# KoslickiLab/YACHT

Measured on AMD Instinct MI355X. Metric: ref-sketch containment queries/sec (yacht run), higher is better.
Workload: dtype u64

## Files before the change

yacht_amd/csrc/yh_api.hip:

```cpp
#include "yh_common.h"
#include "yh_abund.h"
#include "yh_explain.h"
#include "yh_sort.h"
#include "yh_pack.h"

#include <mutex>
#include <unordered_map>

#include <stdarg.h>
#include <string.h>
#include <time.h>

#include <algorithm>
#include <utility>
#include <vector>

static thread_local char g_err[1024] = "";

void yh_set_error(const char* fmt, ...) {
    va_list ap;
    va_start(ap, fmt);
    vsnprintf(g_err, sizeof(g_err), fmt, ap);
    va_end(ap);
}
// ... 546 lines not shown
        return db_create_common(nullptr, v.offsets, false, v.n_refs, device_id, flags, out, &v);
    } catch (const std::bad_alloc&) {
        yh_set_error("yh_db_create_packed: out of host memory");
        return YH_ERR_OOM;
    } catch (const std::exception& ex) {
        yh_set_error("yh_db_create_packed: %s", ex.what());
        return YH_ERR_INVALID_ARG;
    }
}

int yh_db_destroy(yh_db* db) {
    if (!db) return YH_OK;
    if (db->device >= 0) (void)hipSetDevice(db->device);
    if (db->fin_stream) (void)hipStreamSynchronize(db->fin_stream);
    if (db->stream) (void)hipStreamSynchronize(db->stream);
    if (db->ev_fin) (void)hipEventDestroy(db->ev_fin);
    for (yh_db::BatchSlot& bs : db->batch) if (bs.ev_first) (void)hipEventDestroy(bs.ev_first);
    if (db->tmp_psort) { yh_psort_destroy(db, db->tmp_psort); db->tmp_psort = nullptr; }
    if (db->ctx_bits[0]) {
        db->d_maskbits = db->ctx_bits[0];
        db->d_work = db->ctx_work[0];
        db->d_work_count = db->ctx_count[0];
        for (int c = 1; c < YH_RUN_CONTEXTS; ++c) {
            yh_dfree(db, db->ctx_bits[c]);
            yh_dfree(db, db->ctx_work[c]);
            yh_dfree(db, db->ctx_count[c]);
        }
    }
    void* ptrs[] = {db->d_values, db->d_offsets, db->d_sizes, db->d_g, db->d_po, db->d_pr, db->d_pg, db->d_nshared,
                    db->d_dh, db->d_dref, db->d_dir, db->d_bkt, db->d_cbkt, db->d_ovf_keys, db->d_ovf_vals,
                    db->d_rpo, db->d_rg, db->d_rrec, db->d_rrecx, db->d_filter, db->d_hrec, db->d_hrecx, db->d_hmult, db->d_hpo,
                    db->d_work, db->d_work_count, db->d_mask, db->d_maskbits, db->d_hit, db->d_excl_e, db->d_overlap_tmp,
                    db->d_sample_tmp, db->d_out_tmp, db->d_flag, db->d_reps, db->batch[0].d_scratch, db->batch[1].d_scratch, db->batch[2].d_scratch, db->d_sdelta, db->d_shdr, db->d_srec,
                    db->d_wg_key, db->d_ghost_src, db->d_bad_word, db->d_prank, db->d_fz_rec, db->d_fz_list, db->d_fz_list2, db->d_fz_off, db->d_fz_tab};
    for (void* p : ptrs)
        if (p) yh_dfree(db, p);
    for (auto& pair : db->ev_xfer)
        for (hipEvent_t e : pair) if (e) (void)hipEventDestroy(e);
    ring_destroy(db->ev_overlap);
    ring_destroy(db->ev_excl);
    ring_destroy(db->ev_pair);
    for (hipStream_t q : db->st_in) if (q) (void)hipStreamSynchronize(q);
    for (RunSlot& s : db->slots) {
        yh_dfree(db, s.d_sample);
        yh_dfree(db, s.d_packed);
        yh_dfree(db, s.d_rows);
        yh_dfree(db, s.d_out);
        yh_dfree(db, s.d_bad);
        if (s.h_bad) (void)hipHostFree(s.h_bad);
        if (s.ev_up) (void)hipEventDestroy(s.ev_up);
        if (s.ev_out) (void)hipEventDestroy(s.ev_out);
    }
    for (hipStream_t q : db->st_in) if (q) (void)hipStreamDestroy(q);
    if (db->stream) { (void)hipStreamSynchronize(db->stream); yh_pool_trim(db); }
    if (db->own_stream) (void)hipStreamDestroy(db->own_stream);
    free(db->h_pw_i);
    free(db->h_pw_j);
    free(db->h_pw_c);
    delete db;
    return YH_OK;
}

int yh_db_get_info(yh_db* db, yh_db_info* info) {
    if (!db_ok(db)) return YH_ERR_INVALID_ARG;
    if (!info) { yh_set_error("info is null"); return YH_ERR_INVALID_ARG; }
    memset(info, 0, sizeof(*info));
    info->n_refs = db->n_refs;
// ... 1010 lines not shown
```

yacht_amd/csrc/yh_batch.hip:

```cpp
#include "yh_common.h"

#include <stdlib.h>
#include <string.h>

#include <algorithm>
#include <vector>

namespace {

constexpr u32 BATCH_MAX = 256;
constexpr u32 BATCH_MAX_PLANES = BATCH_MAX / 64;
inline u32 planes_of(u32 n_samples) { return (n_samples + 63u) / 64u; }

constexpr int EXCL_BLOCK = 256;
inline u32 grid_for(u64 work_items, u32 block, u32 max_blocks = 16384) {
    u64 g = (work_items + block - 1) / block;
    if (g < 1) g = 1;
    if (g > max_blocks) g = max_blocks;
    return (u32)g;
}

#ifndef YH_BATCH_TILE
#define YH_BATCH_TILE 2048
#endif
constexpr u32 BATCH_TILE = YH_BATCH_TILE;
#ifndef YH_BATCH_U
#define YH_BATCH_U 1
#endif
constexpr int BATCH_U = YH_BATCH_U;

constexpr u32 BATCH_TBITS = 10;
__global__ void __launch_bounds__(256) k_batch_lookup(const u64* __restrict__ samples, const u64* __restrict__ soff,
                                                      u32 n_samples, const YhDirView dv, const u64* __restrict__ po,
                                                      const u32* __restrict__ pr, u64 n_refs,
                                                      u32* __restrict__ overlap , u32* __restrict__ ovsh ,
                                                      const u32* __restrict__ filter, u64 filter_mul) {
    constexpr u32 TSLOTS = 1u << BATCH_TBITS;
    __shared__ u64 off[BATCH_MAX + 1];
    __shared__ u64 s_max_nt;
    __shared__ u32 tkey[TSLOTS], tcnt[TSLOTS], tcnt2[TSLOTS];
    for (u32 q = threadIdx.x; q <= n_samples; q += 256) off[q] = soff[q];
    if (threadIdx.x == 0) s_max_nt = 0;
    __syncthreads();
    {
        u64 m = 0;
        if (threadIdx.x < 64)
            for (u32 q = threadIdx.x; q < n_samples; q += 64) m = max(m, (off[q + 1] - off[q] + BATCH_TILE - 1) / BATCH_TILE);
        if (threadIdx.x < 64 && m) atomicMax((unsigned long long*)&s_max_nt, (unsigned long long)m);
    }
    __syncthreads();
    const u64 max_nt = s_max_nt;
    const u64 n_slots = max_nt * n_samples;
    const u64 group = 8ull * n_samples;
    for (u64 c = blockIdx.x; c < (n_slots + group - 1) / group * group; c += gridDim.x) {
        const u64 l = c % group;
        const u64 v = (c / group) * 8 + (l & 7u);
        const u32 s = (u32)(l >> 3);
        if (v >= max_nt) continue;
        const u64 n_s = off[s + 1] - off[s], nt_s = (n_s + BATCH_TILE - 1) / BATCH_TILE;
        if (nt_s == 0) continue;
        const u64 i = v * nt_s / max_nt;
        if (v > 0 && (v - 1) * nt_s / max_nt == i) continue;
        for (u32 k = threadIdx.x; k < TSLOTS; k += 256) { tkey[k] = 0; tcnt[k] = 0; tcnt2[k] = 0; }
        __syncthreads();
        u32* row = overlap + (u64)s * n_refs;
        u32* row2 = ovsh + (u64)s * n_refs;
        auto add = [&](u32 ref, bool shared) {
#if defined(YH_ABLATE_BATCH) && YH_ABLATE_BATCH
            if (ref == 0x7ffffff1u) row[0] = 1;
            return;
#endif
            u32 slot = (ref * 2654435761u) >> (32 - BATCH_TBITS);
#if defined(YH_BATCH_DIRECT_ATOMICS) && YH_BATCH_DIRECT_ATOMICS
            atomicAdd(&row[ref], 1u);
            if (shared) atomicAdd(&row2[ref], 1u);
            return;
#endif
#pragma unroll 1
            for (int probe = 0; probe < 2; ++probe, slot = (slot + 1) & (TSLOTS - 1)) {
                const u32 old = atomicCAS(&tkey[slot], 0u, ref + 1);
                if (old == 0 || old == ref + 1) {
                    atomicAdd(&tcnt[slot], 1u);
                    if (shared) atomicAdd(&tcnt2[slot], 1u);
                    return;
                }
            }
            atomicAdd(&row[ref], 1u);
            if (shared) atomicAdd(&row2[ref], 1u);
        };
        const u64 k_end = min(n_s, (i + 1) * BATCH_TILE);
        auto hits_of = [&](u32 r) {
            if (r == YH_DIR_NONE) return;
            if (!(r & 0x80000000u)) {
                add(r, false);
            } else {
                const u32 gi = r & 0x7fffffffu;
                for (u64 q = po[gi], qe = po[gi + 1]; q < qe; ++q) add(pr[q], true);
            }
        };
        for (u64 k0 = i * BATCH_TILE; k0 < k_end; k0 += 256u * BATCH_U) {
            u64 h[BATCH_U];
            bool ok[BATCH_U];
            u32 w[BATCH_U];
            u64 bit[BATCH_U];
            YhDirView::v4u a[BATCH_U], b[BATCH_U], c[BATCH_U], d[BATCH_U];
#pragma unroll
            for (int u = 0; u < BATCH_U; ++u) {
                const u64 k = k0 + (u64)u * 256u + threadIdx.x;
#if defined(YH_BATCH_NT) && (YH_BATCH_NT & 2)
                h[u] = __builtin_nontemporal_load(&samples[off[s] + min(k, k_end - 1)]);
#else
                h[u] = samples[off[s] + min(k, k_end - 1)];
#endif
                ok[u] = k < k_end && h[u] <= dv.max_hash;
                if (!ok[u]) h[u] = 0;
            }
#if defined(YH_ABLATE_BATCH_READS) && (YH_ABLATE_BATCH_READS & 2)
            if (false) {
#else
            if (filter) {
#endif
#pragma unroll
                for (int u = 0; u < BATCH_U; ++u) {
                    bit[u] = yh_bucket_of(h[u], dv.bkt_lsh, filter_mul);
                    w[u] = filter[bit[u] >> 5];
                }
#pragma unroll
                for (int u = 0; u < BATCH_U; ++u) {
                    const u32 m = yh_filter_mask(h[u], bit[u]);
                    ok[u] = ok[u] && (w[u] & m) == m;
// ... 408 lines not shown
                   u32* d_overlap, u32* d_excl, u32* d_match, int phases, u64* d_maskword_out, const u64* d_gathered,
                   u32 n_ranks, int slot) {
    if (!db->has_dir || !db->has_index) {
        yh_set_error("yh_run_batch needs the directory of the distinct hashes (handle created with YH_DB_NO_DIRECTORY?)");
        return YH_ERR_UNSUPPORTED;
    }
    if (n_samples < 1 || n_samples > BATCH_MAX) { yh_set_error("1..%u samples per batch", BATCH_MAX); return YH_ERR_INVALID_ARG; }
    const u32 npl = planes_of(n_samples);
    const bool split_streams = db->fin_stream && phases != 3;
    hipStream_t st = (split_streams && phases == 2) ? db->fin_stream : db->stream;
    const u64 N = db->n_refs;
    if (N == 0) return YH_OK;
    const u64 BN = (u64)n_samples * N;
    const u64 G = db->n_shared;
    if (G && db->n_postings && !db->d_hrec) { yh_set_error("yh_run_batch needs the holder sets of the handle"); return YH_ERR_UNSUPPORTED; }
    yh_db::BatchSlot& bs = db->batch[slot];
    u64* d_maskword = nullptr;
    u32* d_ovsh = nullptr;
    u64 need = 0;
    YH_TRY(batch_slot_scratch(db, slot, (phases & 1) ? n_samples : std::max(n_samples, bs.n_samples), &d_maskword, &d_ovsh, &need));
    if (phases & 1) { bs.n_samples = n_samples; bs.words_valid = false; }
    if (phases & 1) {
    YH_HIP(hipMemsetAsync(d_overlap, 0, BN * sizeof(u32), st));
    if (!bs.ovsh_clean) YH_HIP(hipMemsetAsync(bs.d_scratch, 0, bs.cap, st));
    bs.ovsh_clean = false;
    yh_ring_record_begin(db, db->ev_overlap, st);
    if (total_hashes && db->n_distinct) {
        const u64 n_tiles = (total_hashes + BATCH_TILE - 1) / BATCH_TILE + n_samples;
        if (n_tiles >> 31) { yh_set_error("batch too large"); return YH_ERR_INVALID_ARG; }
        static const long grid_env = [] { const char* e = yh_tune_env("YH_BATCH_GRID"); return e ? atol(e) : -1L; }();
        const u64 grid_cap = grid_env < 0 ? 32768ull : grid_env == 0 ? (u64)0x7fffff00 : (u64)grid_env;
        k_batch_lookup<<<(u32)std::min<u64>((n_tiles + 7) / 8 * 8, grid_cap), 256, 0, st>>>(d_samples, d_soff, n_samples, yh_dir_view(db),
                                                                                       db->d_po, db->d_pr, N, d_overlap, d_ovsh,
                                                                                       yh_filter_of(db), db->filter_mul);
    }
    yh_ring_record_end(db, db->ev_overlap, st);
    hipStream_t sw = st;
    if (split_streams) {
        YH_HIP(hipEventRecord(bs.ev_first, st));
        sw = db->fin_stream;
        YH_HIP(hipStreamWaitEvent(sw, bs.ev_first, 0));
    }
    k_batch_maskwords<<<(u32)((N + 255) / 256), 256, 0, sw>>>(d_overlap, n_samples, N, d_maskword, split_streams ? nullptr : db->d_maskbits);
    if (d_maskword_out) YH_HIP(hipMemcpyAsync(d_maskword_out, d_maskword, (u64)npl * N * sizeof(u64), hipMemcpyDeviceToDevice, sw));
    if (split_streams) { YH_HIP(hipEventRecord(db->ev_fin, sw)); db->fin_pending = true; }
    }
    if (!(phases & 2)) { YH_HIP(hipGetLastError()); return YH_OK; }
    YH_HIP(hipMemsetAsync(d_excl, 0, BN * sizeof(u32), st));
    yh_ring_record_begin(db, db->ev_excl, st);
    if (d_gathered)
        k_batch_or_maskwords<<<(u32)((N + 255) / 256), 256, 0, st>>>(d_gathered, n_ranks, N, d_maskword, db->d_maskbits, npl);
    if (G && db->n_postings) {
        YH_HIP(hipMemsetAsync(db->d_work_count, 0, sizeof(u32), st));
        k_batch_worklist<<<(u32)((N + 255) / 256), 256, 0, st>>>(N, db->d_maskbits, db->d_hpo, db->d_work, db->d_work_count);
        const u32 sets_blocks = (u32)std::min<u64>(4096, ((u64)db->n_chunks + 3) / 4 + 1);
        k_batch_sets<<<sets_blocks, 256, 0, st>>>(db->d_work, db->d_work_count, db->d_hrec, db->d_hrecx, db->d_hmult, db->d_pr,
                                                   d_maskword, N, d_excl, npl);
    }
    static const bool dense_final = [] { const char* e = yh_tune_env("YH_BATCH_DENSE_FINAL"); return e && e[0] == '1'; }();
    if (dense_final) {
        k_batch_final<<<grid_for(BN, 256, 8192), 256, 0, st>>>(n_samples, N, db->d_sizes, db->d_nshared, d_overlap, d_ovsh,
                                                               d_excl, d_match, d_gathered ? d_maskword : nullptr);
    } else {
        YH_HIP(hipMemsetAsync(d_match, 0, BN * sizeof(u32), st));
        k_batch_final_sparse<<<(u32)((N + 255) / 256), 256, 0, st>>>(n_samples, N, npl, db->d_sizes, db->d_nshared, d_overlap, d_ovsh,
                                                                   d_excl, d_match, d_maskword);
    }
// ... 27 lines not shown
```

yacht_amd/csrc/yh_build.hip:

```cpp
#include "yh_common.h"
#include "yh_sort.h"
#include "yh_pack.h"

#include <rocprim/device/device_merge.hpp>
#include <rocprim/device/device_radix_sort.hpp>
#include <rocprim/device/device_scan.hpp>
#include <rocprim/iterator/counting_iterator.hpp>
#include <rocprim/iterator/transform_iterator.hpp>

#include <stdio.h>
#include <time.h>

#include <algorithm>
#include <atomic>
#include <thread>
#include <mutex>
#include <vector>

namespace {

constexpr int WAVE = 64;

__global__ void k_scan_refs(const u64* __restrict__ values, const u64* __restrict__ offsets, u64 n_refs,
                            u32* __restrict__ sizes, u32* __restrict__ flag, u64* __restrict__ maxv) {
// ... 324 lines not shown
            atomicAdd(&hcnt[pref[p]], 1u);
        }
    }
}

__global__ void k_chunk_counts(const u32* __restrict__ nshared, u64 n, u32* __restrict__ cc) {
    const u64 r = blockIdx.x * (u64)blockDim.x + threadIdx.x;
    if (r < n) cc[r] = (nshared[r] + (u32)(YH_EXCL_PIECE - 1)) / (u32)YH_EXCL_PIECE;
}
__global__ void k_fill_rg(u64 n_post, const u32* __restrict__ pr, const u32* __restrict__ pg, const u64* __restrict__ po,
                          const u32* __restrict__ rpo, u32* __restrict__ cursor, u32* __restrict__ rg,
                          uint4* __restrict__ rrec, uint4* __restrict__ rrecx, u32* __restrict__ pref) {
    for (u64 k = blockIdx.x * (u64)blockDim.x + threadIdx.x; k < n_post; k += (u64)gridDim.x * blockDim.x) {
        const u32 r = pr[k], g = pg[k];
        const u32 dst = rpo[r] + atomicAdd(&cursor[r], 1u);
        rg[dst] = g;
        if (pref) pref[dst] = r;
        if (rrec) {
            const u64 q0 = po[g], q1 = po[g + 1];
            uint4 rec, recx = make_uint4(0u, 0u, 0u, 0u);
            if (q1 - q0 <= 8) {
                u32 o[7] = {0u, 0u, 0u, 0u, 0u, 0u, 0u};
                u32 n = 0;
                for (u64 q = q0; q < q1; ++q)
                    if (q != k) o[n++] = pr[q];
                rec = make_uint4(o[0], o[1], o[2], n);
                recx = make_uint4(o[3], o[4], o[5], o[6]);
            } else {
                rec = make_uint4((u32)q0, (u32)(q1 - q0), 0u, 0xffffffffu);
            }
            rrec[dst] = rec;
            rrecx[dst] = recx;
        }
    }
}
__global__ void k_filter_build(const u64* __restrict__ dh, u64 n, u32 lsh, u64 fmul, u32* __restrict__ filter) {
    for (u64 i = blockIdx.x * (u64)blockDim.x + threadIdx.x; i < n; i += (u64)gridDim.x * blockDim.x) {
        const u64 bit = __umul64hi(dh[i] << lsh, fmul);
        atomicOr(&filter[bit >> 5], yh_filter_mask(dh[i], bit));
    }
}

inline u32 grid_for(u64 work_items, u32 block, u32 max_blocks = 16384) {
    u64 g = (work_items + block - 1) / block;
    if (g < 1) g = 1;
    if (g > max_blocks) g = max_blocks;
    return (u32)g;
}

}

static int validate_begin(yh_db* db) {
    const u64 N = db->n_refs;
    YH_TRY(yh_dmalloc(db, (void**)&db->d_sizes, std::max<u64>(N, 1) * sizeof(u32)));
    YH_TRY(yh_dmalloc(db, (void**)&db->d_flag, 32));
    YH_HIP(hipMemsetAsync(db->d_flag, 0, 32, db->stream));
    YH_HIP(hipMemsetAsync(db->d_sizes, 0, std::max<u64>(N, 1) * sizeof(u32), db->stream));
    return YH_OK;
}
static int validate_refs(yh_db* db, const u64* d_values, const u64* d_offsets, u64 r0, u64 r1) {
    if (r1 > r0) {
        u64* d_maxv = (u64*)(db->d_flag + 2);
        k_scan_refs<<<grid_for((r1 - r0) * WAVE, 256), 256, 0, db->stream>>>(d_values, d_offsets + r0, r1 - r0, db->d_sizes + r0,
                                                                            db->d_flag, d_maxv);
        YH_HIP(hipGetLastError());
    }
// ... 727 lines not shown
            IDX_HIP(hipMemsetAsync(db->d_ovf_keys, 0, cap * sizeof(u64), st));
            IDX_HIP(hipMemsetAsync(db->d_ovf_vals, 0xff, cap * sizeof(u32), st));
            if (rc == YH_OK)
                k_cbkt_build<<<grid_for(db->n_distinct, 256), 256, 0, st>>>(d_dh_tmp, d_dref_tmp, db->n_distinct, db->bkt_lsh, mul_c,
                                                                            reinterpret_cast<u32*>(db->d_cbkt), db->d_ovf_keys,
                                                                            db->d_ovf_vals, db->ovf_mask);
            IDX_HIP(hipGetLastError());
            static const u32 fbph = [] { const char* e = yh_tune_env("YH_FILTER_BPH"); return e ? (u32)atoi(e) : 4u; }();
            static const u64 fmin = [] { const char* e = yh_tune_env("YH_FILTER_MIN"); return e ? (u64)atoll(e) : (u64)(1u << 20); }();
            if (rc == YH_OK && fbph && db->n_distinct >= fmin) {
                const u64 fbits = ((db->n_distinct * fbph + 511) / 512) * 512;
                db->filter_mul = mul_for(fbits);
                db->filter_bits = fbits;
                rc = yh_dmalloc(db, (void**)&db->d_filter, fbits / 8 + 64);
                IDX_HIP(hipMemsetAsync(db->d_filter, 0, fbits / 8 + 64, st));
                if (rc == YH_OK && db->filter_mul)
                    k_filter_build<<<grid_for(db->n_distinct, 256), 256, 0, st>>>(d_dh_tmp, db->n_distinct, db->bkt_lsh, db->filter_mul,
                                                                                  db->d_filter);
                IDX_HIP(hipGetLastError());
            }
            IDX_HIP(hipStreamSynchronize(st));
        }
        IDX_HIP(hipStreamSynchronize(st));
        TRACE("index: emit + table + filter");
        yh_tfree(db, d_dh_tmp);
        yh_tfree(db, d_dref_tmp);
        if (rc == YH_OK && full) db->has_dir = true;
        if (rc == YH_OK && want_stream) rc = build_stream(db, d_sk, d_sv, d_elem_g, H);
        TRACE("index: delta stream");
        yh_tfree(db, d_elem_g);
        d_elem_g = nullptr;
        IDX_HIP(hipGetLastError());
        IDX_HIP(hipMemcpyAsync(db->d_po + db->n_shared, &db->n_postings, sizeof(u64), hipMemcpyHostToDevice, st));
        if (rc == YH_OK && db->n_postings && N && !(db->flags & YH_DB_PAIRWISE_ONLY)) {
            u32 *d_cc = nullptr, *d_cpo = nullptr, *d_cur = nullptr;
            void* d_st = nullptr;
            size_t st_bytes = 0;
            rc = yh_dmalloc(db, (void**)&db->d_rpo, (N + 1) * sizeof(u32));
            if (rc == YH_OK) rc = yh_dmalloc(db, (void**)&db->d_rg, db->n_postings * sizeof(u32));
            if (rc == YH_OK && want_stream) rc = yh_dmalloc(db, (void**)&db->d_rrec, (db->n_postings + 1) * sizeof(uint4));
            if (rc == YH_OK && want_stream) rc = yh_dmalloc(db, (void**)&db->d_rrecx, (db->n_postings + 1) * sizeof(uint4));
            IDX_HIP(yh_tmalloc(db, (void**)&d_cc, N * sizeof(u32)));
            IDX_HIP(yh_tmalloc(db, (void**)&d_cpo, (N + 1) * sizeof(u32)));
            IDX_HIP(yh_tmalloc(db, (void**)&d_cur, N * sizeof(u32)));
            IDX_HIP(rocprim::inclusive_scan(nullptr, st_bytes, db->d_nshared, db->d_rpo + 1, N, rocprim::plus<u32>(), st));
            IDX_HIP(yh_tmalloc(db, &d_st, st_bytes + 256));
            IDX_HIP(hipMemsetAsync(db->d_rpo, 0, sizeof(u32), st));
            IDX_HIP(hipMemsetAsync(d_cpo, 0, sizeof(u32), st));
            IDX_HIP(hipMemsetAsync(d_cur, 0, N * sizeof(u32), st));
            IDX_HIP(rocprim::inclusive_scan(d_st, st_bytes, db->d_nshared, db->d_rpo + 1, N, rocprim::plus<u32>(), st));
            if (rc == YH_OK) k_chunk_counts<<<(u32)((N + 255) / 256), 256, 0, st>>>(db->d_nshared, N, d_cc);
            IDX_HIP(rocprim::inclusive_scan(d_st, st_bytes, d_cc, d_cpo + 1, N, rocprim::plus<u32>(), st));
            u32 n_chunks = 0;
            IDX_HIP(hipMemcpyAsync(&n_chunks, d_cpo + N, sizeof(u32), hipMemcpyDeviceToHost, st));
            IDX_HIP(hipStreamSynchronize(st));
            db->n_chunks = n_chunks;
            if (rc == YH_OK) rc = yh_dmalloc(db, (void**)&db->d_work, ((u64)n_chunks + 64) * sizeof(uint4));
            if (rc == YH_OK) rc = yh_dmalloc(db, (void**)&db->d_work_count, 16);
            IDX_HIP(hipMemsetAsync(db->d_work_count, 0, 16, st));
            u32* d_pref = nullptr;
            if (want_stream) IDX_HIP(yh_tmalloc(db, (void**)&d_pref, db->n_postings * sizeof(u32)));
            if (rc == YH_OK)
                k_fill_rg<<<grid_for(db->n_postings, 256), 256, 0, st>>>(db->n_postings, db->d_pr, db->d_pg, db->d_po, db->d_rpo,
                                                                         d_cur, db->d_rg, db->d_rrec, db->d_rrecx, d_pref);
            IDX_HIP(hipGetLastError());
            if (trace_on()) { IDX_HIP(hipStreamSynchronize(st)); TRACE("index: reference-major view"); }
// ... 70 lines not shown
```

yacht_amd/csrc/yh_common.h:

```cpp
#pragma once

#include <hip/hip_runtime.h>
#include <stdint.h>
#include <stdio.h>
#include <string>
#include <vector>

#include "../../include/yacht_hip.h"

typedef unsigned long long u64;
typedef uint32_t u32;
typedef uint16_t u16;
typedef uint8_t u8;

static_assert(sizeof(u64) == sizeof(uint64_t), "u64 must be 64 bits");

void yh_set_error(const char* fmt, ...);

#define YH_HIP(call)                                                                        \
    do {                                                                                    \
        hipError_t e__ = (call);                                                            \
        if (e__ != hipSuccess) {                                                            \
            yh_set_error("%s failed: %s (%s:%d)", #call, hipGetErrorString(e__), __FILE__,  \
                         __LINE__);                                                         \
// ... 41 lines not shown
    u64 rows_cap = 0;
    bool rows_mode = false;
    u32* d_out = nullptr;
    u32* d_bad = nullptr;
    u32* h_bad = nullptr;
    u32* h_bad_dev = nullptr;
    hipEvent_t ev_up = nullptr, ev_out = nullptr;
    bool busy = false;
};

struct yh_db {
    int device = -1;
    uint32_t flags = 0;
    hipStream_t own_stream = nullptr;
    hipStream_t stream = nullptr;

    u64 n_refs = 0;
    u64 n_hashes = 0;
    u64 max_hash = 0;
    u64 device_bytes = 0;

    u64* d_values = nullptr;
    u64* d_offsets = nullptr;

    u32* d_sizes = nullptr;

    bool has_index = false;
    u64 n_distinct = 0;
    u64 n_shared = 0;
    u64 n_postings = 0;
    u64* d_g = nullptr;
    u64* d_po = nullptr;
    u32* d_pr = nullptr;
    u32* d_pg = nullptr;
    u32* d_prank = nullptr;
    u32* d_nshared = nullptr;
    bool fz = false;
    u64* d_fz_rec = nullptr;
    u32* d_fz_list = nullptr;
    u32* d_fz_list2 = nullptr;
    u64 fz_list_split = 0;
    u64 n_spilled_pairs = 0, n_spilled_buckets = 0;
    u32 sort_path = 0;
    u64* d_fz_off = nullptr;
    u32* d_fz_tab = nullptr;
    bool fz_nshared = false;

    u64* d_dh = nullptr;
    u32* d_dref = nullptr;
    u32* d_dir = nullptr;
    u32 dir_shift = 0, dir_nb = 0;
    u32* d_rpo = nullptr;
    u32* d_rg = nullptr;
    uint4* d_work = nullptr;
    u32* d_work_count = nullptr;
    uint4* d_rrec = nullptr;
    uint4* d_rrecx = nullptr;
    u32* d_filter = nullptr;
    u64 filter_mul = 0, filter_bits = 0;
    uint4* d_hrec = nullptr;
    uint4* d_hrecx = nullptr;
    u32* d_hmult = nullptr;
    u32* d_hpo = nullptr;
    u32 n_sets = 0;
    u32 n_chunks = 0;
    u8* d_sdelta = nullptr;
// ... 262 lines not shown
```

yacht_amd/csrc/yh_query.hip:

```cpp
#include "yh_common.h"

#include <stdlib.h>
#include <string.h>

#include <algorithm>
#include <vector>

namespace {

constexpr int WAVE = 64;
constexpr int EXCL_PIECE_C = YH_EXCL_PIECE;

typedef u64 u64x2 __attribute__((ext_vector_type(2)));

__device__ __forceinline__ u32 xcd_remap(u32 bid, u32 nwg) {
    const u32 q = nwg >> 3, r = nwg & 7u;
    const u32 xcd = bid & 7u;
    const u32 base = (xcd < r) ? xcd * (q + 1) : r * (q + 1) + (xcd - r) * q;
    return base + (bid >> 3);
}

#ifndef YH_XCD_ATOMICS
#define YH_XCD_ATOMICS 0
#endif
// ... 671 lines not shown
    for (u64 q = q0; q < qe; q += 4) {
        u32 h[4];
#pragma unroll
        for (int i = 0; i < 4; ++i) h[i] = pr[min(q + (u64)i, qe - 1)];
#pragma unroll
        for (int i = 0; i < 4; ++i)
            if (q + (u64)i < qe) add(h[i]);
    }
}

#ifndef YH_IDX_THREADS
#define YH_IDX_THREADS 1024
#endif
#ifndef YH_IDX_TBITS
#define YH_IDX_TBITS 10
#endif
constexpr int IDX_THREADS = YH_IDX_THREADS;
struct TileLookup {
    const u64* sample;
    u64 n;
    YhDirView dv;
    const u32* filter;
    u64 filter_mul;
    const u64* po;
    const u32* pr;
    u32* reps;
    u32 rep_mask;
    u64 n_refs;
    u8* hit;
    u32* reps2;
    u32* work_count;
    const u32* bad;
    u32 bad_gen;
};
template <int U, int THREADS, int TBITS>
__device__ __forceinline__ void lookup_tile_body(u32 wg, u32* tkey, u32* tcnt, u32* tcnt2, const TileLookup& q) {
    constexpr u32 TSLOTS = 1u << TBITS;
    const u64* __restrict__ sample = q.sample;
    const u64 n = q.n;
    const YhDirView& dv = q.dv;
    const u32* __restrict__ filter = q.filter;
    if (q.work_count && wg == 0 && threadIdx.x == 0) *q.work_count = 0;
    u32* my = q.reps + (u64)replica_of(wg, q.rep_mask) * q.n_refs;
    u32* my2 = q.reps2 ? q.reps2 + (u64)replica_of(wg, q.rep_mask) * q.n_refs : nullptr;
    const u64 base = wg * (u64)(THREADS * U);
    u64 h[U];
    bool ok[U];
#pragma unroll
    for (int u = 0; u < U; ++u) {
        const u64 t = base + (u64)u * THREADS + threadIdx.x;
        h[u] = sample[min(t, n - 1)];
        ok[u] = t < n && h[u] <= dv.max_hash;
        if (!ok[u]) h[u] = 0;
    }
#if !(defined(YH_ABLATE_LOOKUP) && (YH_ABLATE_LOOKUP & 32))
    if (q.bad && *q.bad == q.bad_gen) return;
#endif
    for (u32 k = threadIdx.x; k < TSLOTS; k += THREADS) { tkey[k] = 0; tcnt[k] = 0; tcnt2[k] = 0; }
    YhDirView::v4u a[U], b[U], c[U], d[U];
    u32 r[U];
#if defined(YH_ABLATE_LOOKUP) && (YH_ABLATE_LOOKUP & 16)
    if (false) {
#else
    if (filter) {
#endif
        u64 bit[U];
// ... 14 lines not shown
        for (int u = 0; u < U; ++u) {
            a[u] = b[u] = c[u] = d[u] = YhDirView::v4u{0u, 0u, 0u, 0u};
#if defined(YH_ABLATE_LOOKUP) && (YH_ABLATE_LOOKUP & 8)
            ok[u] = ok[u] && h[u] == 0x123456789abcdefull;
#endif
            if (ok[u]) dv.cbkt_request(h[u], a[u], b[u], c[u], d[u]);
        }
#pragma unroll
        for (int u = 0; u < U; ++u) asm volatile("" : "+v"(a[u]), "+v"(b[u]), "+v"(c[u]), "+v"(d[u]));
    }
    __syncthreads();
    auto add = [&](u32 ref, bool shared) {
#if defined(YH_ABLATE_LOOKUP) && (YH_ABLATE_LOOKUP & 4)
        if (ref == 0x7ffffff1u) my[0] = 1;
        return;
#endif
        u32 slot = (ref * 2654435761u) >> (32 - TBITS);
#pragma unroll 1
        for (int probe = 0; probe < 2; ++probe, slot = (slot + 1) & (TSLOTS - 1)) {
            const u32 old = atomicCAS(&tkey[slot], 0u, ref + 1);
            if (old == 0 || old == ref + 1) {
                atomicAdd(&tcnt[slot], 1u);
                if (shared && my2) atomicAdd(&tcnt2[slot], 1u);
                return;
            }
        }
        count_add(&my[ref], 1u);
        if (shared && my2) count_add(&my2[ref], 1u);
    };
#pragma unroll
    for (int u = 0; u < U; ++u) {
        r[u] = YH_DIR_NONE;
        if (ok[u]) r[u] = dv.cbkt ? dv.cbkt_resolve(h[u], a[u], b[u], c[u], d[u]) : dv.find(h[u]);
        if (r[u] == YH_DIR_NONE) continue;
        if (!(r[u] & 0x80000000u)) {
            add(r[u], false);
        } else {
            const u32 gi = r[u] & 0x7fffffffu;
            if (q.hit) q.hit[gi] = 1;
#if !(defined(YH_ABLATE_LOOKUP) && (YH_ABLATE_LOOKUP & 1))
            walk_holders(q.po, q.pr, gi, [&](u32 holder) { add(holder, true); });
#endif
        }
    }
    __syncthreads();
#if defined(YH_ABLATE_LOOKUP) && (YH_ABLATE_LOOKUP & 2)
    if (n == 1) return;
    return;
#endif
    for (u32 k = threadIdx.x; k < TSLOTS; k += THREADS)
        if (tkey[k]) {
            count_add(&my[tkey[k] - 1], tcnt[k]);
            if (my2 && tcnt2[k]) count_add(&my2[tkey[k] - 1], tcnt2[k]);
        }
}

template <int U, int THREADS, int TBITS>
__global__ void __launch_bounds__(THREADS) k_index_lookup_tile(const TileLookup q) {
    constexpr u32 TSLOTS = 1u << TBITS;
    __shared__ u32 tkey[TSLOTS];
    __shared__ u32 tcnt[TSLOTS];
    __shared__ u32 tcnt2[TSLOTS];
    lookup_tile_body<U, THREADS, TBITS>(blockIdx.x, tkey, tcnt, tcnt2, q);
}

constexpr u32 EXCL_PIECE = YH_EXCL_PIECE;
#ifndef YH_EXCL_U
#define YH_EXCL_U 4
#endif
constexpr int EXCL_U = YH_EXCL_U;
constexpr u32 EXCL_LDS_WORDS = 12288;

__device__ __forceinline__ u32 wave_sum(u32 v) {
#pragma unroll
    for (int off = 32; off >= 1; off >>= 1) v += (u32)__shfl_xor((int)v, off);
    return v;
// ... 114 lines not shown
    for (u32 i = threadIdx.x; i < q.n_mask_words / 4; i += blockDim.x) dst[i] = src[i];
    __syncthreads();
}

template <bool LDSMASK, int U = EXCL_U>
__device__ __forceinline__ void excl_pieces_body(u32 wg, u32 n_wgs, u32* lmask, const ExclPieces& q) {
    const u32 WPB = blockDim.x >> 6;
    const u32 n_work = *q.work_count;
    if (wg * WPB >= n_work) return;
    const u32 w0 = wg * WPB + (threadIdx.x >> 6);
    uint4 first_rec = make_uint4(0u, 0u, 0u, 0u);
    if (w0 < n_work) first_rec = q.work[w0];
    if (LDSMASK) stage_subset_bits(lmask, q);
    for (u32 w = w0; w < n_work; w += n_wgs * WPB)
        excl_one_piece<LDSMASK, U>((w == w0) ? first_rec : q.work[w], lmask, q);
}

template <bool LDSMASK>
__global__ void __launch_bounds__(EXCL_PIECE_THREADS) k_excl_pieces(const ExclPieces q) {
    extern __shared__ u32 lmask[];
    excl_pieces_body<LDSMASK>(blockIdx.x, gridDim.x, lmask, q);
}

struct StepFused {
    TileLookup look;   u32 look_wgs;
    u32* r_reps; u32 r_R; u64 r_n; u32* r_out; u32* r_maskbits; FusedRun r_fused; u32 red_wgs;
    ExclPieces excl;   u32 excl_wgs; u32 excl_lds;
};
template <int U, int THREADS, int TBITS>
__global__ void __launch_bounds__(THREADS, THREADS == 1024 ? 8 : 4) k_step_fused(const StepFused s) {
    extern __shared__ u32 smem[];
    constexpr u32 TSLOTS = 1u << TBITS;
    u32 b = blockIdx.x;
#if defined(YH_ABLATE_LOOKUP) && (YH_ABLATE_LOOKUP & 64)
    if (b < s.excl_wgs + s.red_wgs) return;
#endif
    if (b < s.excl_wgs) {
        if (s.excl_lds) excl_pieces_body<true, 2>(b, s.excl_wgs, smem, s.excl);
        else excl_pieces_body<false, 2>(b, s.excl_wgs, smem, s.excl);
        return;
    }
    b -= s.excl_wgs;
    if (b < s.red_wgs) {
        const u32 blocks = (u32)((s.r_n + 4ull * THREADS - 1) / (4ull * THREADS));
        for (u32 blk = b; blk < blocks; blk += s.red_wgs) {
            reduce_replicas_multi<4>(blk, smem, s.r_reps, s.r_R, s.r_n, s.r_out, s.r_maskbits, s.r_fused);
            __syncthreads();
        }
        return;
    }
    b -= s.red_wgs;
    lookup_tile_body<U, THREADS, TBITS>(b, smem, smem + TSLOTS, smem + 2 * TSLOTS, s.look);
}

__global__ void k_excl_final(u64 n, const u8* __restrict__ mask, const u32* __restrict__ sizes,
                             const u32* __restrict__ nshared, const u32* __restrict__ overlap,
                             const u32* __restrict__ ex_e, const u32* __restrict__ ex_m,
                             const u32* __restrict__ ovsh, u32* __restrict__ out_e, u32* __restrict__ out_m,
                             uint4* __restrict__ hit16, u64 n_hit16) {
    const u64 j = blockIdx.x * (u64)blockDim.x + threadIdx.x;
    for (u64 i = j; i < n_hit16; i += (u64)gridDim.x * blockDim.x) hit16[i] = make_uint4(0, 0, 0, 0);
    if (j >= n) return;
    u32 e = 0, m = 0;
    if (mask[j]) {
        e = sizes[j] - nshared[j] + ex_e[j];
        m = overlap[j] - ovsh[j] + ex_m[j];
// ... 170 lines not shown
    yh_ring_record_end(db, db->ev_excl);
    YH_HIP(hipGetLastError());
    return YH_OK;
}

int yh_q_overlap_indexed(yh_db* db, const u64* d_sample, u64 n_sample, u32* d_overlap, bool for_exclusive,
                         u32* d_fused_excl, u32* d_fused_match, u32* d_bits_out, bool lookup_half_only) {
    if (!db->has_dir || !db->has_index) {
        yh_set_error("this handle has no directory of its distinct hashes (YH_DB_NO_DIRECTORY, or no index)");
        return YH_ERR_UNSUPPORTED;
    }
    hipStream_t st = db->stream;
    const u64 N = db->n_refs;
    if (N == 0) return YH_OK;
    u32 R;
    YH_TRY(ensure_reps(db, R));
    static const u32 ri_env = [] { const char* e = yh_tune_env("YH_INDEX_REPS"); return e ? (u32)atoi(e) : 0u; }();
    static const long tile_env = [] { const char* e = yh_tune_env("YH_INDEX_TILE"); return e ? atol(e) : -1L; }();
    int U = n_sample >= 512ull * IDX_THREADS ? 2 : n_sample >= 256ull * IDX_THREADS ? 1 : 256;
    if (tile_env == 1 || tile_env == 2 || tile_env == 4 || tile_env == 256) U = (int)tile_env;
    const u32 r_want = ri_env ? ri_env : 4u;
    while (R > 1 && R > r_want) R >>= 1;
    const bool fused = fused_possible(db, d_fused_excl, for_exclusive);
    if (for_exclusive && db->n_shared && !fused) YH_TRY(claim_hit_flags(db));
    u32* const reps1 = db->d_reps;
    u32* const reps2 = reps1 + db->reps_cap;
    yh_ring_record_begin(db, db->ev_overlap);
    u8* const d_hitflags = (for_exclusive && db->n_shared && !fused) ? db->d_hit : nullptr;
    u32* const d_reps2 = fused ? reps2 : nullptr;
    const u32* const d_filter = yh_filter_of(db);
#define YH_TILE_LAUNCH(UU, TT, BB, FILTER)                                                                                        \
    k_index_lookup_tile<UU, TT, BB><<<(u32)((n_sample + (u64)(TT) * (UU) - 1) / ((u64)(TT) * (UU))), TT, 0, st>>>(                 \
        TileLookup{d_sample, n_sample, yh_dir_view(db), FILTER, db->filter_mul, db->d_po, db->d_pr, reps1, R - 1, N, d_hitflags,    \
                   d_reps2, db->d_work_count, db->d_bad, db->bad_gen})
    if (n_sample && db->n_distinct && U == 256)
        YH_TILE_LAUNCH(1, 256, 8, nullptr);
    else if (n_sample && db->n_distinct && U == 4) YH_TILE_LAUNCH(4, IDX_THREADS, YH_IDX_TBITS, d_filter);
    else if (n_sample && db->n_distinct && U == 2) YH_TILE_LAUNCH(2, IDX_THREADS, YH_IDX_TBITS, d_filter);
    else if (n_sample && db->n_distinct && U == 1) YH_TILE_LAUNCH(1, IDX_THREADS, YH_IDX_TBITS, d_filter);
#undef YH_TILE_LAUNCH
    else if (fused && db->d_work_count)
        YH_HIP(hipMemsetAsync(db->d_work_count, 0, sizeof(u32), st));
    yh_ring_record_end(db, db->ev_overlap);
    k_reduce_replicas<<<(u32)((N + 255) / 256), 256, 0, st>>>(
        reps1, R, N, d_overlap, (for_exclusive && !fused) ? db->d_mask : nullptr,
        for_exclusive ? db->d_maskbits : nullptr, (for_exclusive && !fused) ? db->d_excl_e : nullptr,
        fused ? FusedRun{reps2, db->d_sizes, db->d_nshared, db->range_local ? nullptr : d_fused_excl, d_fused_match, d_bits_out,
                         db->d_hpo, db->range_local ? nullptr : db->d_work, db->d_work_count,
                         (u32)(db->n_ghost ? db->ghost_begin : N)}
              : FusedRun{});
    if (fused && !lookup_half_only) {
        yh_ring_record_begin(db, db->ev_excl);
        if (db->n_chunks) launch_excl_pieces(db, db->d_maskbits, nullptr, d_fused_excl, nullptr, nullptr, true);
        yh_ring_record_end(db, db->ev_excl);
    }
    YH_HIP(hipGetLastError());
    return fused ? 2 : YH_OK;
}

bool yh_q_step_fused_ok(const yh_db* db, u64 n_sample) {
    return db->has_dir && db->has_index && db->d_cbkt && fused_possible(db, reinterpret_cast<const u32*>(db), true) &&
           db->n_chunks && !db->n_ghost && n_sample >= 1 && n_sample <= 0xfffffff0ull;
}
int yh_q_step_fused(yh_db* db, const u64* d_sample, u64 n_sample, u32* d_overlap, u32* d_excl, u32* d_match) {
    hipStream_t st = db->stream;
    const u64 N = db->n_refs;
    u32 R;
    YH_TRY(ensure_reps(db, R));
    while (R > 1 && R > 4u) R >>= 1;
    const int form = !d_sample ? 0 : n_sample >= 512ull * 1024 ? 2 : n_sample >= 256ull * 1024 ? 1 : 0;
    const u32 threads = form ? 1024u : 256u, waves = threads / 64, tslots = form ? 1024u : 256u;
    StepFused s{};
    u32 lds_words = 3 * tslots;
    if (db->pend_excl >= 0) {
        const int c = db->pend_excl;
        s.excl = excl_args(db, db->ctx_count[c], db->ctx_work[c], db->ctx_bits[c], nullptr, db->pend_excl_out, nullptr, nullptr, true);
        s.excl_wgs = std::min<u32>((db->n_chunks + waves - 1) / waves, 4096u / waves);
        s.excl_lds = s.excl.n_mask_words <= EXCL_LDS_WORDS ? 1u : 0u;
        if (s.excl_lds) lds_words = std::max(lds_words, s.excl.n_mask_words);
    }
    if (db->pend_red >= 0) {
        const int c = db->pend_red;
        u32* const reps1 = db->d_reps + (u64)db->pend_red_parity * 2 * db->reps_cap;
        s.r_reps = reps1;
        s.r_R = R;
        s.r_n = N;
        s.r_out = db->pend_red_out[0];
        s.r_maskbits = db->ctx_bits[c];
        s.r_fused = FusedRun{reps1 + db->reps_cap, db->d_sizes, db->d_nshared, db->pend_red_out[1], db->pend_red_out[2], nullptr,
                             db->d_hpo, db->ctx_work[c], db->ctx_count[c], (u32)N};
        s.red_wgs = (u32)((N + 4ull * threads - 1) / (4ull * threads));
    }
    int c_new = -1;
    if (d_sample) {
        c_new = (int)(db->pipe_k % 3);
        const int parity = (int)(db->pipe_k & 1);
        u32* const reps1 = db->d_reps + (u64)parity * 2 * db->reps_cap;
        const u32 per_wg = threads * (form == 2 ? 2u : 1u);
        s.look = TileLookup{d_sample, n_sample, yh_dir_view(db), form ? yh_filter_of(db) : nullptr, db->filter_mul, db->d_po, db->d_pr,
                            reps1, R - 1, N, nullptr, reps1 + db->reps_cap, db->ctx_count[c_new], nullptr, 0u};
        s.look_wgs = (u32)((n_sample + per_wg - 1) / per_wg);
    }
    const u32 total = s.excl_wgs + s.red_wgs + s.look_wgs;
    if (total) {
        if (d_sample) yh_ring_record_begin(db, db->ev_overlap);
        if (form == 2) k_step_fused<2, 1024, 10><<<total, 1024, lds_words * sizeof(u32), st>>>(s);
        else if (form == 1) k_step_fused<1, 1024, 10><<<total, 1024, lds_words * sizeof(u32), st>>>(s);
        else k_step_fused<1, 256, 8><<<total, 256, lds_words * sizeof(u32), st>>>(s);
        if (d_sample) yh_ring_record_end(db, db->ev_overlap);
        YH_HIP(hipGetLastError());
    }
    db->pend_excl = db->pend_red;
    db->pend_excl_out = db->pend_red >= 0 ? db->pend_red_out[1] : nullptr;
    db->pend_red = c_new;
    if (d_sample) {
        db->pend_red_parity = (int)(db->pipe_k & 1);
        db->pend_red_out[0] = d_overlap;
        db->pend_red_out[1] = d_excl;
        db->pend_red_out[2] = d_match;
        db->pipe_last_ctx = c_new;
        ++db->pipe_k;
    }
    return YH_OK;
}

int yh_q_overlap_bsearch(yh_db* db, const u64* d_sample, u64 n_sample, u32* d_overlap) {
    if (!db->d_values) { yh_set_error("yh_overlap_bsearch needs a handle created with YH_DB_KEEP_CSR"); return YH_ERR_UNSUPPORTED; }
    hipStream_t st = db->stream;
    const u64 N = db->n_refs;
    YH_HIP(hipMemsetAsync(d_overlap, 0, std::max<u64>(N, 1) * sizeof(u32), st));
    if (N == 0) return YH_OK;
    k_overlap_bsearch<<<grid_for(N * WAVE, 256, 8192), 256, 0, st>>>(db->d_values, db->d_offsets, N, d_sample, n_sample,
                                                                     d_overlap);
// ... 32 lines not shown
```

Before: 2.533 billion.

## Inline small shared-hash holder lists into 32-byte records for lookup kernels

At build time a per-shared-group 32-byte record is created that stores up to seven holder reference ids inline, or a sentinel when the group has more holders. The batch and tile lookup kernels load this record with two vector loads, issued early to overlap with adding unique hits, in place of the dependent po then pr pointer chase for small groups. This trades extra device memory and a build kernel for fewer dependent global loads. The batch kernel also gains a launch-bounds occupancy hint, and an optional lookup-first block ordering is added behind a macro.

```diff
diff --git a/yacht_amd/csrc/yh_api.hip b/yacht_amd/csrc/yh_api.hip
--- a/yacht_amd/csrc/yh_api.hip
+++ b/yacht_amd/csrc/yh_api.hip
@@ -602,7 +602,7 @@
                     db->d_rpo, db->d_rg, db->d_rrec, db->d_rrecx, db->d_filter, db->d_hrec, db->d_hrecx, db->d_hmult, db->d_hpo,
                     db->d_work, db->d_work_count, db->d_mask, db->d_maskbits, db->d_hit, db->d_excl_e, db->d_overlap_tmp,
                     db->d_sample_tmp, db->d_out_tmp, db->d_flag, db->d_reps, db->batch[0].d_scratch, db->batch[1].d_scratch, db->batch[2].d_scratch, db->d_sdelta, db->d_shdr, db->d_srec,
-                    db->d_wg_key, db->d_ghost_src, db->d_bad_word, db->d_prank, db->d_fz_rec, db->d_fz_list, db->d_fz_list2, db->d_fz_off, db->d_fz_tab};
+                    db->d_wg_key, db->d_ghost_src, db->d_bad_word, db->d_prank, db->d_fz_rec, db->d_fz_list, db->d_fz_list2, db->d_fz_off, db->d_fz_tab, db->d_ghold};
     for (void* p : ptrs)
         if (p) yh_dfree(db, p);
     for (auto& pair : db->ev_xfer)
diff --git a/yacht_amd/csrc/yh_batch.hip b/yacht_amd/csrc/yh_batch.hip
--- a/yacht_amd/csrc/yh_batch.hip
+++ b/yacht_amd/csrc/yh_batch.hip
@@ -30,11 +30,12 @@
 constexpr int BATCH_U = YH_BATCH_U;
 
 constexpr u32 BATCH_TBITS = 10;
-__global__ void __launch_bounds__(256) k_batch_lookup(const u64* __restrict__ samples, const u64* __restrict__ soff,
-                                                      u32 n_samples, const YhDirView dv, const u64* __restrict__ po,
-                                                      const u32* __restrict__ pr, u64 n_refs,
-                                                      u32* __restrict__ overlap , u32* __restrict__ ovsh ,
-                                                      const u32* __restrict__ filter, u64 filter_mul) {
+__global__ void __launch_bounds__(256, 8) k_batch_lookup(const u64* __restrict__ samples, const u64* __restrict__ soff,
+                                                         u32 n_samples, const YhDirView dv, const u64* __restrict__ po,
+                                                         const u32* __restrict__ pr, u64 n_refs,
+                                                         u32* __restrict__ overlap , u32* __restrict__ ovsh ,
+                                                         const u32* __restrict__ filter, u64 filter_mul,
+                                                         const uint4* __restrict__ ghold) {
     constexpr u32 TSLOTS = 1u << BATCH_TBITS;
     __shared__ u64 off[BATCH_MAX + 1];
     __shared__ u64 s_max_nt;
@@ -95,7 +96,20 @@
                 add(r, false);
             } else {
                 const u32 gi = r & 0x7fffffffu;
-                for (u64 q = po[gi], qe = po[gi + 1]; q < qe; ++q) add(pr[q], true);
+                YhDirView::v4u ga{0xffffffffu, 0u, 0u, 0u}, gb{0u, 0u, 0u, 0u};
+                if (ghold) {
+                    const YhDirView::v4u* p = reinterpret_cast<const YhDirView::v4u*>(ghold) + 2 * (u64)gi;
+                    ga = p[0]; gb = p[1];
+                    asm volatile("" : "+v"(ga), "+v"(gb));
+                }
+                if (ga.x != 0xffffffffu) {
+                    const u32 hid[7] = {ga.y, ga.z, ga.w, gb.x, gb.y, gb.z, gb.w};
+#pragma unroll
+                    for (int t = 0; t < 7; ++t)
+                        if ((u32)t < ga.x) add(hid[t], true);
+                } else {
+                    for (u64 q = po[gi], qe = po[gi + 1]; q < qe; ++q) add(pr[q], true);
+                }
             }
         };
         for (u64 k0 = i * BATCH_TILE; k0 < k_end; k0 += 256u * BATCH_U) {
@@ -570,7 +584,7 @@
         const u64 grid_cap = grid_env < 0 ? 32768ull : grid_env == 0 ? (u64)0x7fffff00 : (u64)grid_env;
         k_batch_lookup<<<(u32)std::min<u64>((n_tiles + 7) / 8 * 8, grid_cap), 256, 0, st>>>(d_samples, d_soff, n_samples, yh_dir_view(db),
                                                                                        db->d_po, db->d_pr, N, d_overlap, d_ovsh,
-                                                                                       yh_filter_of(db), db->filter_mul);
+                                                                                       yh_filter_of(db), db->filter_mul, db->d_ghold);
     }
     yh_ring_record_end(db, db->ev_overlap, st);
     hipStream_t sw = st;
diff --git a/yacht_amd/csrc/yh_build.hip b/yacht_amd/csrc/yh_build.hip
--- a/yacht_amd/csrc/yh_build.hip
+++ b/yacht_amd/csrc/yh_build.hip
@@ -380,6 +380,22 @@
             rrec[dst] = rec;
             rrecx[dst] = recx;
         }
+    }
+}
+__global__ void k_holder_records(u64 G, const u64* __restrict__ po, const u32* __restrict__ pr, uint4* __restrict__ ghold) {
+    for (u64 g = blockIdx.x * (u64)blockDim.x + threadIdx.x; g < G; g += (u64)gridDim.x * blockDim.x) {
+        const u64 q0 = po[g], q1 = po[g + 1];
+        uint4 lo = make_uint4(0xffffffffu, 0xffffffffu, 0xffffffffu, 0xffffffffu), hi = lo;
+        if (q1 - q0 <= 7) {
+            u32 h[7] = {0u, 0u, 0u, 0u, 0u, 0u, 0u};
+#pragma unroll
+            for (int i = 0; i < 7; ++i)
+                if (q0 + (u64)i < q1) h[i] = pr[q0 + (u64)i];
+            lo = make_uint4((u32)(q1 - q0), h[0], h[1], h[2]);
+            hi = make_uint4(h[3], h[4], h[5], h[6]);
+        }
+        ghold[2 * g] = lo;
+        ghold[2 * g + 1] = hi;
     }
 }
 __global__ void k_filter_build(const u64* __restrict__ dh, u64 n, u32 lsh, u64 fmul, u32* __restrict__ filter) {
@@ -1173,6 +1189,12 @@
         d_elem_g = nullptr;
         IDX_HIP(hipGetLastError());
         IDX_HIP(hipMemcpyAsync(db->d_po + db->n_shared, &db->n_postings, sizeof(u64), hipMemcpyHostToDevice, st));
+        static const bool no_ghold = [] { const char* e = yh_tune_env("YH_NO_HOLDER_RECORDS"); return e && e[0] == '1'; }();
+        if (rc == YH_OK && full && db->n_shared && !no_ghold) {
+            rc = yh_dmalloc(db, (void**)&db->d_ghold, 2 * db->n_shared * sizeof(uint4));
+            if (rc == YH_OK) k_holder_records<<<grid_for(db->n_shared, 256), 256, 0, st>>>(db->n_shared, db->d_po, db->d_pr, db->d_ghold);
+            IDX_HIP(hipGetLastError());
+        }
         if (rc == YH_OK && db->n_postings && N && !(db->flags & YH_DB_PAIRWISE_ONLY)) {
             u32 *d_cc = nullptr, *d_cpo = nullptr, *d_cur = nullptr;
             void* d_st = nullptr;
diff --git a/yacht_amd/csrc/yh_common.h b/yacht_amd/csrc/yh_common.h
--- a/yacht_amd/csrc/yh_common.h
+++ b/yacht_amd/csrc/yh_common.h
@@ -97,6 +97,7 @@
     u64* d_g = nullptr;
     u64* d_po = nullptr;
     u32* d_pr = nullptr;
+    uint4* d_ghold = nullptr;
     u32* d_pg = nullptr;
     u32* d_prank = nullptr;
     u32* d_nshared = nullptr;
diff --git a/yacht_amd/csrc/yh_query.hip b/yacht_amd/csrc/yh_query.hip
--- a/yacht_amd/csrc/yh_query.hip
+++ b/yacht_amd/csrc/yh_query.hip
@@ -727,6 +727,7 @@
     u32* work_count;
     const u32* bad;
     u32 bad_gen;
+    const uint4* ghold;
 };
 template <int U, int THREADS, int TBITS>
 __device__ __forceinline__ void lookup_tile_body(u32 wg, u32* tkey, u32* tcnt, u32* tcnt2, const TileLookup& q) {
@@ -807,16 +808,39 @@
     for (int u = 0; u < U; ++u) {
         r[u] = YH_DIR_NONE;
         if (ok[u]) r[u] = dv.cbkt ? dv.cbkt_resolve(h[u], a[u], b[u], c[u], d[u]) : dv.find(h[u]);
-        if (r[u] == YH_DIR_NONE) continue;
-        if (!(r[u] & 0x80000000u)) {
-            add(r[u], false);
+    }
+    YhDirView::v4u ga[U], gb[U];
+#pragma unroll
+    for (int u = 0; u < U; ++u) {
+        ga[u] = YhDirView::v4u{0xffffffffu, 0u, 0u, 0u};
+        gb[u] = YhDirView::v4u{0u, 0u, 0u, 0u};
+#if !(defined(YH_ABLATE_LOOKUP) && (YH_ABLATE_LOOKUP & 1))
+        if (q.ghold && r[u] != YH_DIR_NONE && (r[u] & 0x80000000u)) {
+            const YhDirView::v4u* p = reinterpret_cast<const YhDirView::v4u*>(q.ghold) + 2 * (u64)(r[u] & 0x7fffffffu);
+            ga[u] = p[0]; gb[u] = p[1];
+        }
+#endif
+    }
+#pragma unroll
+    for (int u = 0; u < U; ++u)
+        if (r[u] != YH_DIR_NONE && !(r[u] & 0x80000000u)) add(r[u], false);
+#pragma unroll
+    for (int u = 0; u < U; ++u) asm volatile("" : "+v"(ga[u]), "+v"(gb[u]));
+#pragma unroll
+    for (int u = 0; u < U; ++u) {
+        if (r[u] == YH_DIR_NONE || !(r[u] & 0x80000000u)) continue;
+        const u32 gi = r[u] & 0x7fffffffu;
+        if (q.hit) q.hit[gi] = 1;
+#if !(defined(YH_ABLATE_LOOKUP) && (YH_ABLATE_LOOKUP & 1))
+        if (ga[u].x != 0xffffffffu) {
+            const u32 hid[7] = {ga[u].y, ga[u].z, ga[u].w, gb[u].x, gb[u].y, gb[u].z, gb[u].w};
+#pragma unroll
+            for (int t = 0; t < 7; ++t)
+                if ((u32)t < ga[u].x) add(hid[t], true);
         } else {
-            const u32 gi = r[u] & 0x7fffffffu;
-            if (q.hit) q.hit[gi] = 1;
-#if !(defined(YH_ABLATE_LOOKUP) && (YH_ABLATE_LOOKUP & 1))
             walk_holders(q.po, q.pr, gi, [&](u32 holder) { add(holder, true); });
-#endif
-        }
+        }
+#endif
     }
     __syncthreads();
 #if defined(YH_ABLATE_LOOKUP) && (YH_ABLATE_LOOKUP & 2)
@@ -997,6 +1021,9 @@
     extern __shared__ u32 smem[];
     constexpr u32 TSLOTS = 1u << TBITS;
     u32 b = blockIdx.x;
+#if defined(YH_STEP_LOOKUP_FIRST) && YH_STEP_LOOKUP_FIRST
+    b = b < s.look_wgs ? b + s.excl_wgs + s.red_wgs : b - s.look_wgs;
+#endif
 #if defined(YH_ABLATE_LOOKUP) && (YH_ABLATE_LOOKUP & 64)
     if (b < s.excl_wgs + s.red_wgs) return;
 #endif
@@ -1233,7 +1260,7 @@
 #define YH_TILE_LAUNCH(UU, TT, BB, FILTER)                                                                                        \
     k_index_lookup_tile<UU, TT, BB><<<(u32)((n_sample + (u64)(TT) * (UU) - 1) / ((u64)(TT) * (UU))), TT, 0, st>>>(                 \
         TileLookup{d_sample, n_sample, yh_dir_view(db), FILTER, db->filter_mul, db->d_po, db->d_pr, reps1, R - 1, N, d_hitflags,    \
-                   d_reps2, db->d_work_count, db->d_bad, db->bad_gen})
+                   d_reps2, db->d_work_count, db->d_bad, db->bad_gen, db->d_ghold})
     if (n_sample && db->n_distinct && U == 256)
         YH_TILE_LAUNCH(1, 256, 8, nullptr);
     else if (n_sample && db->n_distinct && U == 4) YH_TILE_LAUNCH(4, IDX_THREADS, YH_IDX_TBITS, d_filter);
@@ -1299,7 +1326,7 @@
         u32* const reps1 = db->d_reps + (u64)parity * 2 * db->reps_cap;
         const u32 per_wg = threads * (form == 2 ? 2u : 1u);
         s.look = TileLookup{d_sample, n_sample, yh_dir_view(db), form ? yh_filter_of(db) : nullptr, db->filter_mul, db->d_po, db->d_pr,
-                            reps1, R - 1, N, nullptr, reps1 + db->reps_cap, db->ctx_count[c_new], nullptr, 0u};
+                            reps1, R - 1, N, nullptr, reps1 + db->reps_cap, db->ctx_count[c_new], nullptr, 0u, db->d_ghold};
         s.look_wgs = (u32)((n_sample + per_wg - 1) / per_wg);
     }
     const u32 total = s.excl_wgs + s.red_wgs + s.look_wgs;
```

Result: slower. 2.491 billion (-1.7%).
